# Gumo-A/hnsw_rs

Measured on AMD Instinct MI355X. Metric: queries/sec at recall@10>=0.99, 1M x 100d L2, higher is better.
Workload: dtype f32

## Files before the change

### hnsw_rs_amd/csrc/search_lean.hip

```cpp

#include <algorithm>
#include <cstdlib>

#include "device_index.h"
#include "launch.h"
#include "search_common.h"
#include "switches.h"

namespace hx {
namespace {

#define HX_LIKELY(x) __builtin_expect(!!(x), 1)
#define HX_UNLIKELY(x) __builtin_expect(!!(x), 0)

constexpr u64 LK_INVALID = ~0ull;
constexpr u64 LK_MASK = 0x7FFFFFFFFFFFFFFFull;
constexpr u64 LK_EXPANDED = 1ull << 63;

struct LeanArgs {
    const float *rows;
    const uint32_t *adj0;
    const uint32_t *adj_up;
    const uint32_t *upper_base;
    const uint32_t *ovf_off, *ovf_nbrs;
    const float *Q;
    const uint32_t *qsel;
    uint32_t *out_ids;
    float *out_dists;
    uint32_t *out_counts;
    hnsw_query_stats *out_stats;
    uint32_t n_points, ep, nb_layers, S0, S1, ef, n, slots_log2;
    unsigned long long *dbg;
    uint32_t *spill_tab;
    uint32_t spill_log2;
    uint32_t lds_limit;
};

#ifdef HX_STAMPS
__device__ __forceinline__ unsigned long long stamp_now() {
    __builtin_amdgcn_sched_barrier(0);
    asm volatile("s_waitcnt vmcnt(0) lgkmcnt(0)" ::: "memory");
    const unsigned long long t = __builtin_readcyclecounter();
    asm volatile("s_waitcnt lgkmcnt(0)" ::: "memory");
    __builtin_amdgcn_sched_barrier(0);
    return t;
}
#define STAMP(var) const unsigned long long var = stamp_now()
#define STAMP_ADD(slot, a, b) dbg_acc[slot] += (b) - (a)
#ifdef HX_STAMPS_FRONT
constexpr int HX_LEAN_DBG_SLOTS = 50;
#define FSTAMP(var) STAMP(var)
#define FSTAMP_ADD(slot, a, b) STAMP_ADD(slot, a, b)
#define FSTAMP_LDS(var)                                   \
    asm volatile("s_waitcnt lgkmcnt(0)" ::: "memory");   \
    const unsigned long long var = __builtin_readcyclecounter(); \
    asm volatile("s_waitcnt lgkmcnt(0)" ::: "memory")
#define FSTAMP_SINCE_BEGIN(slot) dbg_acc[slot] = __builtin_readcyclecounter() - t_begin
#else
constexpr int HX_LEAN_DBG_SLOTS = 40;
#endif
#define MERGE_DBG_PARAM , unsigned long long *dbg = nullptr
#define MERGE_DBG_ARG(first) , dbg_acc + (first)
#define MERGE_STAMP(var) const unsigned long long var = dbg ? stamp_now() : 0ull
#define MERGE_ADD(off, v) \
    do {                  \
        if (dbg) dbg[off] += (v); \
    } while (0)
#else
#define STAMP(var)
#define STAMP_ADD(slot, a, b)
#define MERGE_DBG_PARAM
#define MERGE_DBG_ARG(first)
#define MERGE_STAMP(var)
#define MERGE_ADD(off, v)
#endif
#if !defined(HX_STAMPS) || !defined(HX_STAMPS_FRONT)
#define FSTAMP(var)
#define FSTAMP_ADD(slot, a, b)
#define FSTAMP_LDS(var)
#define FSTAMP_SINCE_BEGIN(slot)
#endif

__device__ __forceinline__ uint32_t rdlane(uint32_t v, uint32_t l) {
    return (uint32_t)__builtin_amdgcn_readlane((int)v, (int)l);
}
__device__ __forceinline__ u64 rdlane64(u64 v, uint32_t l) {
    return ((u64)rdlane((uint32_t)(v >> 32), l) << 32) | rdlane((uint32_t)v, l);
}
__device__ __forceinline__ uint32_t uni(uint32_t x) { return (uint32_t)__builtin_amdgcn_readfirstlane((int)x); }
__device__ __forceinline__ void lds_fence() { asm volatile("s_waitcnt lgkmcnt(0)" ::: "memory"); }
template <int CTRL>
__device__ __forceinline__ uint32_t dpp_or_max(uint32_t x) {
    return (uint32_t)__builtin_amdgcn_update_dpp(-1, (int)x, CTRL, 0xF, 0xF, false);
}
__device__ __forceinline__ uint32_t wave_min_u32(uint32_t v) {
    v = min(v, dpp_or_max<0xB1>(v));
    v = min(v, dpp_or_max<0x4E>(v));
    v = min(v, dpp_or_max<0x141>(v));
    v = min(v, dpp_or_max<0x140>(v));
    return min(min(rdlane(v, 0), rdlane(v, 16)), min(rdlane(v, 32), rdlane(v, 48)));
}

struct Visited {
    uint32_t *tab;
    uint32_t bshift, bmask;

    __device__ __forceinline__ uint32_t home(uint32_t id) const { return (id * 0x9E3779B1u) >> bshift; }

    __device__ __forceinline__ uint32_t look(uint32_t id, uint32_t b) const {
        const uint4 bk = *reinterpret_cast<const uint4 *>(tab + 4 * b);
        const uint32_t m = min(min(bk.x ^ id, bk.y ^ id), min(bk.z ^ id, bk.w ^ id));
        const uint32_t nf = 4u + (uint32_t)(((int32_t)bk.x >> 31) + ((int32_t)bk.y >> 31) + ((int32_t)bk.z >> 31) +
                                            ((int32_t)bk.w >> 31));
        return m == 0 ? 4u : (nf == 4u ? 5u : nf);
    }
    __device__ __forceinline__ uint32_t claim(uint32_t id, uint32_t b, uint32_t t) const {
        uint32_t old = 0;
        if (t < 4u) old = atomicCAS(tab + 4 * b + t, HX_EMPTY_SLOT, id);
        return old;
    }
    __device__ __forceinline__ bool finish(uint32_t id, uint32_t b, uint32_t t, bool pend, bool fresh) const {
        while (__ballot(pend)) {
            if (pend) {
                if (t == 5u) b = (b + 1) & bmask;
                t = look(id, b);
                const uint32_t old = claim(id, b, t);
                const bool won = old == HX_EMPTY_SLOT;
                fresh |= won;
                pend = (t != 4u) & !won;
            }
        }
        return fresh;
    }
    __device__ __forceinline__ bool insert(uint32_t id, bool ins) const {
        const uint32_t b = home(id);
        uint32_t t = look(id, b);
        t = ins ? t : 4u;
        const uint32_t old = claim(id, b, t);
        const bool fresh = old == HX_EMPTY_SLOT;
        return finish(id, b, t, (t != 4u) & !fresh, fresh);
    }
    __device__ __forceinline__ void clear(uint32_t nslots, int lane) const {
        for (uint32_t s = lane; s < (nslots >> 2); s += 64)
            reinterpret_cast<uint4 *>(tab)[s] = make_uint4(HX_EMPTY_SLOT, HX_EMPTY_SLOT, HX_EMPTY_SLOT, HX_EMPTY_SLOT);
        lds_fence();
    }

    uint32_t *gtab = nullptr;
    uint32_t gshift = 0, gmask = 0;
    bool spill = false;

    __device__ __forceinline__ bool g_contains(uint32_t id) const {
        uint32_t s = ((id * 0x9E3779B1u) >> gshift) & gmask;
        while (true) {
            const uint32_t cur = __hip_atomic_load(gtab + s, __ATOMIC_RELAXED, __HIP_MEMORY_SCOPE_AGENT);
            if (cur == id) return true;
            if (cur == HX_EMPTY_SLOT) return false;
            s = (s + 1) & gmask;
        }
    }
    __device__ __forceinline__ uint32_t g_claim(uint32_t id) const {
        uint32_t s = ((id * 0x9E3779B1u) >> gshift) & gmask;
        while (true) {
            const uint32_t old = atomicCAS(gtab + s, HX_EMPTY_SLOT, id);
            if (old == HX_EMPTY_SLOT) return HX_EMPTY_SLOT;
            if (old == id) return id;
            s = (s + 1) & gmask;
        }
    }
    __device__ __forceinline__ void open_second_level(int lane) {
        const uint32_t nslots = gmask + 1;
        for (uint32_t s = lane; s < (nslots >> 2); s += 64)
            reinterpret_cast<uint4 *>(gtab)[s] = make_uint4(HX_EMPTY_SLOT, HX_EMPTY_SLOT, HX_EMPTY_SLOT, HX_EMPTY_SLOT);
        __builtin_amdgcn_fence(__ATOMIC_RELEASE, "agent");
        asm volatile("s_waitcnt vmcnt(0)" ::: "memory");
        spill = true;
    }
    __device__ __forceinline__ uint32_t look2(uint32_t id, uint32_t b, bool probe, bool claim_now) const {
        uint32_t t = look(id, b);
        if (!spill) return t;
        if (!probe) return 4u;
        while (t == 5u) {
            b = (b + 1) & bmask;
            t = look(id, b);
        }
        if (t == 4u) return 4u;
        if (claim_now) return g_claim(id) == HX_EMPTY_SLOT ? 7u : 4u;
        return g_contains(id) ? 4u : 6u;
    }
    __device__ __forceinline__ uint32_t claim2(uint32_t id, uint32_t b, uint32_t t) const {
        uint32_t old = 0;
        if (t < 4u)
            old = atomicCAS(tab + 4 * b + t, HX_EMPTY_SLOT, id);
        else if (t == 6u)
            old = g_claim(id);
        else if (t == 7u)
            old = HX_EMPTY_SLOT;
        return old;
    }
    __device__ __forceinline__ bool finish2(uint32_t id, uint32_t b, uint32_t t, bool pend, bool fresh) const {
        while (__ballot(pend)) {
            if (pend) {
                if (t == 5u) b = (b + 1) & bmask;
                t = look2(id, b, true, false);
                const uint32_t old = claim2(id, b, t);
                const bool won = old == HX_EMPTY_SLOT;
                fresh |= won;
                pend = (t != 4u) & !won;
            }
        }
        return fresh;
    }
};

#ifndef HX_MERGE_SHIFT_MAX
#define HX_MERGE_SHIFT_MAX 2
#endif
__device__ __forceinline__ void stage_survivors(u64 key, bool surv, u64 smask, uint32_t m, u64 *perm) {
    const uint32_t rk = __builtin_amdgcn_mbcnt_hi((uint32_t)(smask >> 32), __builtin_amdgcn_mbcnt_lo((uint32_t)smask, 0u));
    if (surv) perm[rk] = key;
    if (surv && rk + 1 == m) perm[m] = LK_INVALID;
    asm volatile("" ::: "memory");
}
template <int R>
struct Lst {
    static constexpr int NR = R;
    struct Masks {
        u64 U[R];
    };
    u64 L[R];
    uint32_t n_cur;
    u64 last_key;

    static __device__ __forceinline__ uint32_t idx_of(int r, int lane) { return (uint32_t)(R * lane + r); }
    __device__ __forceinline__ void set_first(u64 key, int lane) {
        if (lane == 0) L[0] = key;
        n_cur = 1;
    }

    __device__ __forceinline__ void init() {
#pragma unroll
        for (int r = 0; r < R; r++) L[r] = LK_INVALID;
        n_cur = 0;
        last_key = LK_INVALID;
    }
    __device__ __forceinline__ int first_unexp() const {
        uint32_t pos = 0xFFFFFFFFu;
#pragma unroll
        for (int r = 0; r < R; r++) {
            const u64 U = __ballot((int32_t)(uint32_t)(L[r] >> 32) >= 0);
            const uint32_t i = U ? (uint32_t)(R * (__ffsll((long long)U) - 1) + r) : 0xFFFFFFFFu;
            pos = min(pos, i);
        }
        return (int)pos;
    }
    __device__ __forceinline__ void unexp_masks(Masks &mk) const {
#pragma unroll
        for (int r = 0; r < R; r++) mk.U[r] = __ballot((int32_t)(uint32_t)(L[r] >> 32) >= 0);
    }
    __device__ __forceinline__ int take_first(Masks &mk) const {
        u64(&U)[R] = mk.U;
        uint32_t pos = 0xFFFFFFFFu;
#pragma unroll
        for (int r = 0; r < R; r++) {
            const uint32_t i = U[r] ? (uint32_t)(R * (__ffsll((long long)U[r]) - 1) + r) : 0xFFFFFFFFu;
            pos = min(pos, i);
        }
#pragma unroll
        for (int r = 0; r < R; r++)
            if (pos != 0xFFFFFFFFu && (pos % R) == (uint32_t)r) U[r] &= U[r] - 1;
        return (int)pos;
    }
    __device__ __forceinline__ uint32_t id_at(uint32_t pos) const {
        uint32_t v = 0;
#pragma unroll
        for (int r = 0; r < R; r++) {
            const uint32_t t = rdlane((uint32_t)L[r], pos / R);
            if ((pos % R) == (uint32_t)r) v = t;
        }
        return v;
    }
    __device__ __forceinline__ u64 key_at(uint32_t pos) const {
        u64 v = 0;
#pragma unroll
        for (int r = 0; r < R; r++) {
            const u64 t = rdlane64(L[r], pos / R);
            if ((pos % R) == (uint32_t)r) v = t;
        }
        return v;
    }
    __device__ __forceinline__ void mark(uint32_t pos, int lane) {
#pragma unroll
        for (int r = 0; r < R; r++)
            if ((pos % R) == (uint32_t)r && (uint32_t)lane == pos / R) L[r] |= LK_EXPANDED;
    }
    __device__ __forceinline__ void refresh_last(uint32_t ef) {
        last_key = n_cur >= ef ? (key_at(ef - 1) & LK_MASK) : LK_INVALID;
    }

    __device__ __forceinline__ void merge(u64 key, uint32_t ef, u64 *perm, int lane MERGE_DBG_PARAM) {
        const bool surv = key < last_key;
        const u64 smask = __ballot(surv);
        if (smask == 0) return;
        const uint32_t m = (uint32_t)__popcll(smask);
        MERGE_STAMP(m0);
        if (m <= HX_MERGE_SHIFT_MAX) {
            u64 it = smask;
            while (it) {
                const uint32_t j = (uint32_t)__ffsll((long long)it) - 1;
                it &= it - 1;
                const u64 e = rdlane64(key, j);
                const uint32_t plo = (uint32_t)__builtin_amdgcn_update_dpp(0, (int)(uint32_t)L[R - 1], 0x138, 0xF, 0xF, false);
                const uint32_t phi = (uint32_t)__builtin_amdgcn_update_dpp(0, (int)(uint32_t)(L[R - 1] >> 32), 0x138, 0xF, 0xF, false);
                const u64 below = ((u64)phi << 32) | plo;
                bool g[R];
#pragma unroll
                for (int r = 0; r < R; r++) g[r] = (L[r] & LK_MASK) > e;
                const bool gb = (below & LK_MASK) > e;
#pragma unroll
                for (int r = R - 1; r >= 0; r--) {
                    const u64 from = r > 0 ? L[r > 0 ? r - 1 : 0] : below;
                    const bool gp = r > 0 ? g[r > 0 ? r - 1 : 0] : gb;
                    L[r] = g[r] ? (gp ? from : e) : L[r];
                }
            }
            n_cur = min(n_cur + m, ef);
            if (ef < 64u * R) {
#pragma unroll
                for (int r = 0; r < R; r++)
                    if ((uint32_t)(R * lane + r) >= ef) L[r] = LK_INVALID;
            }
            refresh_last(ef);
            MERGE_STAMP(m1);
            MERGE_ADD(2, m1 - m0);
            return;
        }
        u64 *sv = perm + 64 * R;
        u64 Lm[R];
        uint32_t shift[R];
#pragma unroll
        for (int r = 0; r < R; r++) {
            Lm[r] = L[r] & LK_MASK;
            shift[r] = 0;
        }
        uint32_t srank = 0;
        stage_survivors(key, surv, smask, m, perm);
        {
            const ulonglong2 *st = reinterpret_cast<const ulonglong2 *>(perm);
            const uint32_t trips = (m + 1) >> 1;
            ulonglong2 e = st[0];
            for (uint32_t t = 1; t < trips; t++) {
                const ulonglong2 nx = st[t];
#pragma unroll
                for (int r = 0; r < R; r++) shift[r] += (e.x < Lm[r] ? 1u : 0u) + (e.y < Lm[r] ? 1u : 0u);
                srank += (e.x < key ? 1u : 0u) + (e.y < key ? 1u : 0u);
                e = nx;
            }
#pragma unroll
            for (int r = 0; r < R; r++) shift[r] += (e.x < Lm[r] ? 1u : 0u) + (e.y < Lm[r] ? 1u : 0u);
            srank += (e.x < key ? 1u : 0u) + (e.y < key ? 1u : 0u);
        }
        asm volatile("" ::: "memory");
        MERGE_STAMP(m2);
        MERGE_ADD(0, m2 - m0);
        const uint32_t n_new = min(n_cur + m, ef);
#pragma unroll
        for (int r = 0; r < R; r++) perm[R * lane + r] = LK_INVALID;
        asm volatile("" ::: "memory");
#pragma unroll
        for (int r = 0; r < R; r++) {
            const uint32_t idx = (uint32_t)(R * lane + r);
            const uint32_t np = idx + shift[r];
            if (idx < n_cur && np < n_new) perm[np] = L[r];
        }
        if (surv) sv[srank] = key;
        asm volatile("" ::: "memory");
        u64 v[R], H[R];
        bool hole[R];
#pragma unroll
        for (int r = 0; r < R; r++) v[r] = perm[R * lane + r];
#pragma unroll
        for (int r = 0; r < R; r++) {
            hole[r] = v[r] == LK_INVALID && (uint32_t)(R * lane + r) < n_new;
            H[r] = __ballot(hole[r]);
        }
#pragma unroll
        for (int r = 0; r < R; r++) {
            uint32_t hr = 0;
#pragma unroll
            for (int r2 = 0; r2 < R; r2++) {
                hr += __builtin_amdgcn_mbcnt_hi((uint32_t)(H[r2] >> 32), __builtin_amdgcn_mbcnt_lo((uint32_t)H[r2], 0u));
                if (r2 < r && hole[r2]) hr++;
            }
            if (hole[r]) v[r] = sv[hr];
        }
#pragma unroll
        for (int r = 0; r < R; r++) L[r] = v[r];
        n_cur = n_new;
        lds_fence();
        refresh_last(ef);
        MERGE_STAMP(m3);
        MERGE_ADD(1, m3 - m2);
        MERGE_ADD(3, m);
        MERGE_ADD(4, 1);
    }
};

struct LstHT {
    static constexpr int NR = 2;
    struct Masks {
        u64 head, tail;
        bool tail_known;
    };
    u64 L[2];
    uint32_t n_cur;
    u64 last_key;

    static __device__ __forceinline__ uint32_t idx_of(int r, int lane) { return (uint32_t)(64 * r + lane); }
    __device__ __forceinline__ void init() {
        L[0] = L[1] = LK_INVALID;
        n_cur = 0;
        last_key = LK_INVALID;
    }
    __device__ __forceinline__ void set_first(u64 key, int lane) {
        if (lane == 0) L[0] = key;
        n_cur = 1;
    }
    __device__ __forceinline__ void unexp_masks(Masks &mk) const {
        mk.head = __ballot((int32_t)(uint32_t)(L[0] >> 32) >= 0);
        mk.tail = 0;
        mk.tail_known = false;
    }
    __device__ __forceinline__ int take_first(Masks &mk) const {
        if (HX_LIKELY(mk.head != 0)) {
            const int pos = __ffsll((long long)mk.head) - 1;
            mk.head &= mk.head - 1;
            return pos;
        }
        if (!mk.tail_known) {
            mk.tail = n_cur > 64 ? __ballot((int32_t)(uint32_t)(L[1] >> 32) >= 0) : 0ull;
            mk.tail_known = true;
        }
        if (mk.tail == 0) return -1;
        const int pos = __ffsll((long long)mk.tail) - 1;
        mk.tail &= mk.tail - 1;
        return 64 + pos;
    }
    __device__ __forceinline__ uint32_t id_at(uint32_t pos) const {
        const uint32_t a = rdlane((uint32_t)L[0], pos & 63u), b = rdlane((uint32_t)L[1], pos & 63u);
        return pos < 64u ? a : b;
    }
    __device__ __forceinline__ u64 key_at(uint32_t pos) const {
        const u64 a = rdlane64(L[0], pos & 63u), b = rdlane64(L[1], pos & 63u);
        return pos < 64u ? a : b;
    }
    __device__ __forceinline__ void mark(uint32_t pos, int lane) {
        if ((uint32_t)lane == pos) L[0] |= LK_EXPANDED;
        if ((uint32_t)lane + 64u == pos) L[1] |= LK_EXPANDED;
    }
    __device__ __forceinline__ void refresh_last(uint32_t ef) {
        last_key = n_cur >= ef ? (rdlane64(L[1], (ef - 65u) & 63u) & LK_MASK) : LK_INVALID;
    }
    static __device__ __forceinline__ u64 shr1(u64 v) {
        const uint32_t lo = (uint32_t)__builtin_amdgcn_update_dpp(0, (int)(uint32_t)v, 0x138, 0xF, 0xF, false);
        const uint32_t hi = (uint32_t)__builtin_amdgcn_update_dpp(0, (int)(uint32_t)(v >> 32), 0x138, 0xF, 0xF, false);
        return ((u64)hi << 32) | lo;
    }
    static __device__ __forceinline__ u64 shr1_behind(u64 v, u64 w) {
        const int wlo = __builtin_amdgcn_update_dpp(0, (int)(uint32_t)w, 0x13C, 0xF, 0xF, false);
        const int whi = __builtin_amdgcn_update_dpp(0, (int)(uint32_t)(w >> 32), 0x13C, 0xF, 0xF, false);
        const uint32_t lo = (uint32_t)__builtin_amdgcn_update_dpp(wlo, (int)(uint32_t)v, 0x138, 0xF, 0xF, false);
        const uint32_t hi = (uint32_t)__builtin_amdgcn_update_dpp(whi, (int)(uint32_t)(v >> 32), 0x138, 0xF, 0xF, false);
        return ((u64)hi << 32) | lo;
    }

    __device__ __forceinline__ void merge(u64 key, uint32_t ef, u64 *perm, int lane MERGE_DBG_PARAM) {
        const bool surv = key < last_key;
        const u64 smask = __ballot(surv);
        if (smask == 0) return;
        const uint32_t m = (uint32_t)__popcll(smask);
        MERGE_STAMP(m0);
        if (m <= HX_MERGE_SHIFT_MAX) {
            u64 it = smask;
            while (it) {
                const uint32_t j = (uint32_t)__ffsll((long long)it) - 1;
                it &= it - 1;
                const u64 e = rdlane64(key, j);
                const u64 b0 = shr1(L[0]), b1 = shr1_behind(L[1], L[0]);
                const bool g0 = (L[0] & LK_MASK) > e, p0 = (b0 & LK_MASK) > e;
                const bool g1 = (L[1] & LK_MASK) > e, p1 = (b1 & LK_MASK) > e;
                L[0] = g0 ? (p0 ? b0 : e) : L[0];
                L[1] = g1 ? (p1 ? b1 : e) : L[1];
            }
            n_cur = min(n_cur + m, ef);
            if (64u + (uint32_t)lane >= ef) L[1] = LK_INVALID;
            refresh_last(ef);
            MERGE_STAMP(m1);
            MERGE_ADD(2, m1 - m0);
            return;
        }
        u64 *sv = perm + 128;
        const u64 Mm = L[0] & LK_MASK, Tm = L[1] & LK_MASK;
        uint32_t sh0 = 0, sh1 = 0, srank = 0;
        stage_survivors(key, surv, smask, m, perm);
        {
            const ulonglong2 *st = reinterpret_cast<const ulonglong2 *>(perm);
            const uint32_t trips = (m + 1) >> 1;
            ulonglong2 e = st[0];
            for (uint32_t t = 1; t < trips; t++) {
                const ulonglong2 nx = st[t];
                sh0 += (e.x < Mm ? 1u : 0u) + (e.y < Mm ? 1u : 0u);
                sh1 += (e.x < Tm ? 1u : 0u) + (e.y < Tm ? 1u : 0u);
                srank += (e.x < key ? 1u : 0u) + (e.y < key ? 1u : 0u);
                e = nx;
            }
            sh0 += (e.x < Mm ? 1u : 0u) + (e.y < Mm ? 1u : 0u);
            sh1 += (e.x < Tm ? 1u : 0u) + (e.y < Tm ? 1u : 0u);
            srank += (e.x < key ? 1u : 0u) + (e.y < key ? 1u : 0u);
        }
        asm volatile("" ::: "memory");
        MERGE_STAMP(m2);
        MERGE_ADD(0, m2 - m0);
        const uint32_t n_new = min(n_cur + m, ef);
        perm[lane] = LK_INVALID;
        perm[64 + lane] = LK_INVALID;
        asm volatile("" ::: "memory");
        {
            const uint32_t i0 = (uint32_t)lane, i1 = 64u + (uint32_t)lane;
            if (i0 < n_cur && i0 + sh0 < n_new) perm[i0 + sh0] = L[0];
            if (i1 < n_cur && i1 + sh1 < n_new) perm[i1 + sh1] = L[1];
        }
        if (surv) sv[srank] = key;
        asm volatile("" ::: "memory");
        u64 v0 = perm[lane], v1 = perm[64 + lane];
        const bool hole0 = v0 == LK_INVALID && (uint32_t)lane < n_new;
        const bool hole1 = v1 == LK_INVALID && 64u + (uint32_t)lane < n_new;
        const u64 H0 = __ballot(hole0), H1 = __ballot(hole1);
        const uint32_t hr0 = __builtin_amdgcn_mbcnt_hi((uint32_t)(H0 >> 32), __builtin_amdgcn_mbcnt_lo((uint32_t)H0, 0u));
        const uint32_t hr1 = (uint32_t)__popcll(H0) +
                             __builtin_amdgcn_mbcnt_hi((uint32_t)(H1 >> 32), __builtin_amdgcn_mbcnt_lo((uint32_t)H1, 0u));
        if (hole0) v0 = sv[hr0];
        if (hole1) v1 = sv[hr1];
        L[0] = v0;
        L[1] = v1;
        n_cur = n_new;
        lds_fence();
        refresh_last(ef);
        MERGE_STAMP(m3);
        MERGE_ADD(1, m3 - m2);
        MERGE_ADD(3, m);
        MERGE_ADD(4, 1);
    }
};

template <int DS>
__device__ __forceinline__ float chain_sum(const uint4 (&w)[DS / 4], const float (&qv)[DS]) {
    float s = 0.0f;
#pragma unroll
    for (int p = 0; p < DS / 4; p++) {
        const uint32_t dw[4] = {w[p].x, w[p].y, w[p].z, w[p].w};
#pragma unroll
        for (int j = 0; j < 4; j += 2) {
            const f32x2 x = {__builtin_bit_cast(float, dw[j]), __builtin_bit_cast(float, dw[j + 1])};
            const f32x2 y = {qv[4 * p + j], qv[4 * p + j + 1]};
            const f32x2 t = x - y;
            const f32x2 t2 = t * t;
            s += t2.x;
            s += t2.y;
        }
    }
    return s;
}
template <int DS>
__device__ __forceinline__ float row_dist(const float *rows, uint32_t id, bool want, const float (&qv)[DS]) {
    float s = 0.0f;
    if (want) {
        const uint4 *src = reinterpret_cast<const uint4 *>(rows + (size_t)id * DS);
        uint4 w[DS / 4];
#pragma unroll
        for (int p = 0; p < DS / 4; p++) w[p] = src[p];
        __builtin_amdgcn_sched_barrier(0);
        s = chain_sum<DS>(w, qv);
    }
    return __builtin_sqrtf(s);
}
__device__ __forceinline__ u64 walk_winner(uint32_t nb, bool fresh, float dist, uint32_t &j) {
    const uint32_t db = fresh ? __builtin_bit_cast(uint32_t, dist) : 0xFFFFFFFFu;
    const uint32_t mn = wave_min_u32(db);
    u64 tie = __ballot(fresh && db == mn);
    j = (uint32_t)__ffsll((long long)tie) - 1;
    uint32_t bid = rdlane(nb, j);
    tie &= tie - 1;
    while (tie) {
        const uint32_t j2 = (uint32_t)__ffsll((long long)tie) - 1;
        tie &= tie - 1;
        const uint32_t id2 = rdlane(nb, j2);
        if (id2 < bid) {
            bid = id2;
            j = j2;
        }
    }
    return ((u64)mn << 32) | bid;
}

typedef float QueryPiece __attribute__((ext_vector_type(4), aligned(4)));
template <int DS>
__device__ __forceinline__ bool load_query_f32(const float *qp, float (&qv)[DS], int lane) {
    static_assert(DS % 4 == 0 && DS / 4 <= 64, "one 16-byte piece per lane in the NaN scan");
    typedef const __attribute__((address_space(1))) QueryPiece *GlobalPieces;
    GlobalPieces src = (GlobalPieces) reinterpret_cast<const QueryPiece *>(qp);
    const QueryPiece mine = src[min(lane, DS / 4 - 1)];
    asm volatile("" : "+v"(src));
#pragma unroll
    for (int p = 0; p < DS / 4; p++) {
        const QueryPiece t = src[p];
#pragma unroll
        for (int j = 0; j < 4; j++) qv[4 * p + j] = t[j];
    }
    const bool bad = (mine[0] != mine[0]) | (mine[1] != mine[1]) | (mine[2] != mine[2]) | (mine[3] != mine[3]);
    const bool ok = __ballot(bad) == 0;
#pragma unroll
    for (int e = 0; e < DS; e++) asm volatile("" : "+v"(qv[e]));
    return ok;
}

struct TableLimits {
    uint32_t lds, all;
};
template <bool SPILLV>
__device__ __forceinline__ TableLimits layer0_table(const LeanArgs &a, Visited &vis, uint32_t hslots, uint32_t cur, int lane) {
    vis.bshift = 32 - (a.slots_log2 - 2);
    vis.bmask = (hslots >> 2) - 1;
    TableLimits lim;
    lim.lds = hslots - (hslots >> 2);
    lim.all = lim.lds;
    if constexpr (SPILLV) {
        if (a.spill_tab != nullptr) {
            if (a.lds_limit != 0) lim.lds = min(lim.lds, max(128u, a.lds_limit));
            vis.gtab = a.spill_tab + ((size_t)blockIdx.x << a.spill_log2);
            vis.gmask = (1u << a.spill_log2) - 1;
            vis.gshift = 32 - a.spill_log2;
            lim.all = lim.lds + (1u << a.spill_log2) / 2;
        }
    }
    vis.clear(hslots, lane);
    vis.insert(cur, lane == 0);
    return lim;
}

template <class LT>
__device__ __forceinline__ void write_results(const LeanArgs &a, uint32_t q, const LT &lst, uint32_t count, int lane) {
#pragma unroll
    for (int r = 0; r < LT::NR; r++) {
        const uint32_t idx = LT::idx_of(r, lane);
        if (idx < a.n) {
            const bool have = idx < count;
            a.out_ids[(size_t)q * a.n + idx] = have ? (uint32_t)lst.L[r] : HX_EMPTY_SLOT;
            if (a.out_dists)
                a.out_dists[(size_t)q * a.n + idx] =
                    have ? __builtin_bit_cast(float, (uint32_t)((lst.L[r] & LK_MASK) >> 32)) : __builtin_inff();
        }
    }
    for (uint32_t idx = 64u * LT::NR + lane; idx < a.n; idx += 64) {
        a.out_ids[(size_t)q * a.n + idx] = HX_EMPTY_SLOT;
        if (a.out_dists) a.out_dists[(size_t)q * a.n + idx] = __builtin_inff();
    }
    if (lane == 0 && a.out_counts) a.out_counts[q] = count;
}
__device__ __forceinline__ void write_stats(const LeanArgs &a, uint32_t q, uint32_t n_dist, uint32_t n_exp, uint32_t sum_deg,
                                            int32_t status, int lane) {
    if (lane == 0) {
        hnsw_query_stats st;
        st.n_dist = n_dist;
        st.n_exp = n_exp;
        st.sum_deg = sum_deg;
        st.status = status;
        a.out_stats[q] = st;
    }
}

template <int DS, class LT, int CK = 4>
__global__ void __launch_bounds__(64) hx_lean_f32_kernel(const LeanArgs a) {
    constexpr int R = LT::NR;
    static_assert(DS % 4 == 0, "whole 16-byte pieces");
    constexpr bool COOP = coop_rows<HNSW_VEC_F32, DS>();
    constexpr bool SPILLV = R >= 6;
    constexpr bool MISS_AHEAD = !COOP && !SPILLV;
    constexpr bool MISS_KEEP = MISS_AHEAD && R <= 2;
    constexpr bool WALK_AHEAD = !COOP && R <= 2;
    extern __shared__ __attribute__((aligned(16))) unsigned char smem[];
    const int lane = threadIdx.x;
    const uint32_t q = a.qsel ? a.qsel[blockIdx.x] : blockIdx.x;
    const uint32_t hslots = 1u << a.slots_log2;
    u64 *perm = reinterpret_cast<u64 *>(smem + 4ull * hslots);
    unsigned char *coop_img = reinterpret_cast<unsigned char *>(perm);
    uint32_t *coop_ids = reinterpret_cast<uint32_t *>(coop_img + HX_COOP_IMG_BYTES);
    Visited vis;
    vis.tab = reinterpret_cast<uint32_t *>(smem);

    uint32_t n_dist = 0, n_exp = 0, sum_deg = 0, n_vis = 0;
    int32_t status = HNSW_OK;
#ifdef HX_STAMPS
    unsigned long long dbg_acc[HX_LEAN_DBG_SLOTS] = {};
    const unsigned long long t_begin = __builtin_readcyclecounter();
    bool dbg_follow = false, dbg_took_pre = false;
    uint32_t dbg_pred_c = HX_EMPTY_SLOT, dbg_pred_p = HX_EMPTY_SLOT, dbg_old_p = HX_EMPTY_SLOT;
#endif

    auto row_ahead = [&](uint32_t id, uint32_t base, int layer) __attribute__((always_inline)) -> uint32_t {
        const bool up = layer >= 1, has = base != HX_EMPTY_SLOT;
        const size_t r = up ? (size_t)(has ? base : 0u) + (uint32_t)max(layer, 1) - 1 : (size_t)id;
        const uint32_t *src = (up ? a.adj_up + r * a.S1 : a.adj0 + r * a.S0) + lane;
        const bool mine = (uint32_t)lane < (up ? (has ? a.S1 : 0u) : min(a.S0, 32u));
        uint32_t v = HX_EMPTY_SLOT;
        if (mine) v = *src;
        return v;
    };
    uint32_t ub_cur = HX_EMPTY_SLOT;
    bool have_ub = false;
    if constexpr (WALK_AHEAD) {
        if (a.ep < a.n_points) {
            ub_cur = a.upper_base[a.ep];
            have_ub = true;
        }
    }

    QueryRegs<DS> qreg;
    float(&qv)[DS] = qreg.v;
    if (!load_query_f32<DS>(a.Q + (size_t)q * DS, qv, lane)) status = HNSW_ERR_NAN_INPUT;
    FSTAMP_SINCE_BEGIN(40);

    auto dist_of = [&](uint32_t id, bool want) __attribute__((always_inline)) -> float {
        if constexpr (COOP) {
            return __builtin_sqrtf(f32_rows_coop<DS, CK, true, true>(reinterpret_cast<const uint8_t *>(a.rows), id, want, qreg,
                                                                    coop_ids, coop_img, lane));
        } else {
            return row_dist<DS>(a.rows, id, want, qv);
        }
    };

    u64 best = LK_INVALID;
    uint32_t cur = a.ep;
    uint32_t row_now = HX_EMPTY_SLOT;
    if (status == HNSW_OK) {
        if (cur >= a.n_points) {
            status = HNSW_ERR_ARG;
        } else {
            if constexpr (WALK_AHEAD) row_now = row_ahead(cur, ub_cur, max((int)a.nb_layers - 1, 0));
            const float d0 = dist_of(cur, lane == 0);
            const uint32_t bits = rdlane(__builtin_bit_cast(uint32_t, d0), 0);
            n_dist = 1;
            if (__builtin_bit_cast(float, bits) != __builtin_bit_cast(float, bits))
                status = HNSW_ERR_NAN_INPUT;
            else
                best = ((u64)bits << 32) | cur;
        }
    }
    struct WalkLane {
        bool fresh;
        uint32_t ubn;
        float dist;
    };
    auto walk_eval = [&](uint32_t id, bool act) __attribute__((always_inline)) -> WalkLane {
        WalkLane r = {false, HX_EMPTY_SLOT, 0.0f};
        if constexpr (WALK_AHEAD) {
            FSTAMP(w0);
            const uint32_t vb = vis.home(id);
            const uint32_t vt0 = vis.look(id, vb);
            const uint32_t vt = act ? vt0 : 4u;
            FSTAMP(w1);
            FSTAMP_ADD(43, w0, w1);
            if (vt != 4u) {
                r.ubn = a.upper_base[id];
                const uint4 *src = reinterpret_cast<const uint4 *>(a.rows + (size_t)id * DS);
                uint4 w[DS / 4];
#pragma unroll
                for (int p = 0; p < DS / 4; p++) w[p] = src[p];
                __builtin_amdgcn_sched_barrier(0);
                const uint32_t old = vis.claim(id, vb, vt);
                r.fresh = old == HX_EMPTY_SLOT;
                const bool pend = !r.fresh;
                if (HX_UNLIKELY(__ballot(pend) != 0)) r.fresh = vis.finish(id, vb, vt, pend, r.fresh);
                __builtin_amdgcn_sched_barrier(0);
                FSTAMP_LDS(g0);
                FSTAMP(g1);
                FSTAMP_ADD(43, w1, g0);
                FSTAMP_ADD(44, g0, g1);
                r.dist = __builtin_sqrtf(chain_sum<DS>(w, qv));
                FSTAMP(g2);
                FSTAMP_ADD(45, g1, g2);
            }
        } else {
            r.fresh = vis.insert(id, act);
            if (HX_LIKELY(__ballot(r.fresh) != 0)) {
                if (r.fresh) r.ubn = a.upper_base[id];
                r.dist = dist_of(id, r.fresh);
            }
        }
        return r;
    };

#ifdef HX_STAMPS
    dbg_acc[25] = __builtin_readcyclecounter() - t_begin;
#endif
    const uint32_t up_slots = max(hslots >> 2, 64u);
    for (int layer = (int)a.nb_layers - 1; layer >= 1 && status == HNSW_OK; layer--) {
        FSTAMP(l0);
        vis.bshift = 32 - (__ffs((int)up_slots) - 1 - 2);
        vis.bmask = (up_slots >> 2) - 1;
        const uint32_t vis_limit = up_slots - (up_slots >> 2);
        vis.clear(up_slots, lane);
        vis.insert(cur, lane == 0);
        n_vis = 1;
        FSTAMP(l1);
        FSTAMP_ADD(41, l0, l1);
        if (!have_ub) {
            ub_cur = uni(a.upper_base[cur]);
            have_ub = true;
        }
        while (status == HNSW_OK) {
            if (ub_cur == HX_EMPTY_SLOT) {
                status = HNSW_ERR_NODE_NOT_IN_GRAPH;
                break;
            }
            n_exp++;
            FSTAMP_LDS(x0);
            FSTAMP(x1);
            FSTAMP_ADD(42, x0, x1);
            FSTAMP_ADD(48, 0, 1);
            bool improved = false;
            uint32_t new_cur = cur, new_ub = ub_cur;
            uint32_t ovf_lo = 0, ovf_hi = 0;
            bool first = true;
            while (true) {
                uint32_t nb = HX_EMPTY_SLOT;
                if (first) {
                    if constexpr (WALK_AHEAD) {
                        nb = row_now;
                    } else {
                        if ((uint32_t)lane < a.S1) nb = a.adj_up[((size_t)ub_cur + (uint32_t)layer - 1) * a.S1 + lane];
                    }
                } else {
                    if (ovf_lo + lane < ovf_hi) nb = a.ovf_nbrs[ovf_lo + lane];
                    ovf_lo += 64;
                }
                const bool valid = (int32_t)nb >= 0;
                if (first) {
                    const u64 pm = __ballot((int32_t)nb < 0 && nb != HX_EMPTY_SLOT);
                    if (HX_UNLIKELY(pm != 0)) {
                        const uint32_t o = rdlane(nb, (uint32_t)__ffsll((long long)pm) - 1) & ~HX_OVF_FLAG;
                        ovf_lo = uni(a.ovf_off[o]);
                        ovf_hi = uni(a.ovf_off[o + 1]);
                    }
                    first = false;
                }
                const uint32_t cnt = (uint32_t)__popcll(__ballot(valid));
                sum_deg += cnt;
                if (HX_LIKELY(cnt != 0)) {
                    if (HX_UNLIKELY(n_vis + cnt > vis_limit)) {
                        status = HNSW_ERR_OVERFLOW;
                        break;
                    }
                    const WalkLane wl = walk_eval(nb, valid);
                    const bool fresh = wl.fresh;
                    const float dist = wl.dist;
                    const u64 fm = __ballot(fresh);
                    const uint32_t nf = (uint32_t)__popcll(fm);
                    n_vis += nf;
                    n_dist += nf;
                    if (HX_LIKELY(fm != 0)) {
                        const bool nan = fresh && dist != dist;
                        if (HX_UNLIKELY(__ballot(nan) != 0)) {
                            status = HNSW_ERR_NAN_INPUT;
                            break;
                        }
                        uint32_t j;
                        const u64 k = walk_winner(nb, fresh, dist, j);
                        if (k < best) {
                            best = k;
                            new_cur = (uint32_t)k;
                            new_ub = rdlane(wl.ubn, j);
                            improved = true;
                        }
                    }
                }
                if (HX_LIKELY(ovf_lo >= ovf_hi)) break;
            }
            if (!improved || status != HNSW_OK) break;
            cur = new_cur;
            ub_cur = new_ub;
            if constexpr (WALK_AHEAD) row_now = row_ahead(cur, ub_cur, layer);
        }
        if constexpr (WALK_AHEAD) row_now = row_ahead(cur, ub_cur, layer - 1);
    }

#ifdef HX_STAMPS
    dbg_acc[7] = __builtin_readcyclecounter() - t_begin;
#endif
    const uint32_t ef = max(1u, a.ef);
    LT lst;
    lst.init();
    if (status == HNSW_OK) {
        FSTAMP(t0);
        const TableLimits lim = layer0_table<SPILLV>(a, vis, hslots, cur, lane);
        FSTAMP(t1);
        FSTAMP_ADD(47, t0, t1);
        const uint32_t lds_limit = lim.lds, vis_limit = lim.all;
        n_vis = 1;
        lst.set_first(best, lane);
        lst.refresh_last(ef);
        const uint32_t S0 = a.S0;
        const bool upper = lane >= 32;
        const uint32_t slot = (uint32_t)lane & 31u;
        uint32_t pre_nb = HX_EMPTY_SLOT, pre_c = HX_EMPTY_SLOT, pre_p = HX_EMPTY_SLOT;
        if constexpr (WALK_AHEAD) {
            pre_nb = row_now;
            pre_c = cur;
        }
        bool carry = false;
        float kdist = 0.0f;

        uint32_t ovf_lo = 0, ovf_hi = 0;

        while (true) {
            STAMP(f0);
            if constexpr (SPILLV) {
                if (HX_UNLIKELY(!vis.spill && vis.gtab != nullptr && n_vis + 64u > lds_limit)) vis.open_second_level(lane);
            }
            int ppos = -1;
            uint32_t pid = HX_EMPTY_SLOT;
            u64 pkey = 0;
            bool kept = false;
            uint32_t nb = HX_EMPTY_SLOT;
            const bool ovf_pass = ovf_lo < ovf_hi;
            if (HX_UNLIKELY(ovf_pass)) {
                if (lane < 32 && ovf_lo + (uint32_t)lane < ovf_hi) nb = a.ovf_nbrs[ovf_lo + (uint32_t)lane];
                ovf_lo += 32;
            } else {
                typename LT::Masks U;
                lst.unexp_masks(U);
                const int cpos = lst.take_first(U);
                if (HX_UNLIKELY(cpos < 0)) break;
                ppos = lst.take_first(U);
                const uint32_t cid = lst.id_at((uint32_t)cpos);
                if constexpr (MISS_AHEAD) {
                    if (ppos >= 0) {
                        pkey = lst.key_at((uint32_t)ppos);
                        pid = (uint32_t)pkey;
                    }
                } else {
                    if (ppos >= 0) pid = lst.id_at((uint32_t)ppos);
                }
                lst.mark((uint32_t)cpos, lane);
                n_exp++;
#ifdef HX_STAMPS
                if (dbg_follow) {
                    if (cid == dbg_pred_c && pid == dbg_pred_p) dbg_acc[19]++;
                    if (pid == dbg_old_p) dbg_acc[20]++;
                    dbg_follow = false;
                }
                dbg_took_pre = pre_c == cid && pre_p == pid;
#endif
                if (HX_LIKELY(pre_c == cid && pre_p == pid)) {
                    nb = pre_nb;
                    if constexpr (MISS_KEEP) kept = carry;
                } else {
                    if (slot < S0 && (!upper || ppos >= 0)) nb = a.adj0[(size_t)(upper ? pid : cid) * S0 + slot];
                }
                pre_c = HX_EMPTY_SLOT;
                carry = false;
            }
#ifdef HX_STAMPS
            asm volatile("s_waitcnt vmcnt(0)" ::: "memory");
            dbg_acc[6]++;
#endif
            STAMP(f1);
            STAMP_ADD(0, f0, f1);
#ifdef HX_STAMPS
            if (!ovf_pass && dbg_took_pre) {
                dbg_acc[21] += f1 - f0;
                dbg_acc[22]++;
            }
#endif
            const u64 pm = ovf_pass ? 0ull : __ballot((int32_t)nb < -1);
            const bool spec_ok = ppos >= 0 && (pm >> 32) == 0;
            const bool valid = (int32_t)nb >= 0 && (!upper || spec_ok);
            const uint32_t vb = vis.home(nb);
            uint32_t vt0;
            if constexpr (SPILLV)
                vt0 = vis.look2(nb, vb, valid, valid && !upper);
            else
                vt0 = vis.look(nb, vb);
            const uint32_t vt = valid ? vt0 : 4u;
            const bool want_pre = vt != 4u;
            const uint32_t ct = upper ? 4u : vt;
            bool fresh = false;
            const bool keptl = MISS_KEEP && kept && upper;
            float dist = keptl ? kdist : 0.0f;
            if constexpr (COOP) {
                const uint32_t old = SPILLV ? vis.claim2(nb, vb, ct) : vis.claim(nb, vb, ct);
                fresh = old == HX_EMPTY_SLOT;
                const bool pend = (ct != 4u) & !fresh;
                if (HX_UNLIKELY(__ballot(pend) != 0)) fresh = SPILLV ? vis.finish2(nb, vb, ct, pend, fresh) : vis.finish(nb, vb, ct, pend, fresh);
                dist = dist_of(nb, upper ? want_pre : fresh);
            } else if (want_pre && !keptl) {
                const uint4 *src = reinterpret_cast<const uint4 *>(a.rows + (size_t)nb * DS);
                uint4 w[DS / 4];
#pragma unroll
                for (int p = 0; p < DS / 4; p++) w[p] = src[p];
                __builtin_amdgcn_sched_barrier(0);
                const uint32_t old = SPILLV ? vis.claim2(nb, vb, ct) : vis.claim(nb, vb, ct);
                fresh = old == HX_EMPTY_SLOT;
                const bool pend = (ct != 4u) & !fresh;
                if (HX_UNLIKELY(__ballot(pend) != 0)) {
                    fresh = SPILLV ? vis.finish2(nb, vb, ct, pend, fresh) : vis.finish(nb, vb, ct, pend, fresh);
#ifdef HX_STAMPS
                    dbg_acc[11]++;
#endif
                }
                __builtin_amdgcn_sched_barrier(0);
#ifdef HX_STAMPS
                __builtin_amdgcn_sched_barrier(0);
                asm volatile("s_waitcnt lgkmcnt(0)" ::: "memory");
                const unsigned long long g0 = __builtin_readcyclecounter();
                asm volatile("s_waitcnt lgkmcnt(0)" ::: "memory");
                const unsigned long long g1 = stamp_now();
                dbg_acc[2] += g1 - g0;
#endif
                const float s = chain_sum<DS>(w, qv);
                dist = __builtin_sqrtf(s);
#ifdef HX_STAMPS
                asm volatile("" ::"v"(dist) : "memory");
                dbg_acc[3] += stamp_now() - g1;
#endif
            }
            const bool want = upper ? want_pre : fresh;
            const u64 vmask = __ballot(valid), fmask = __ballot(fresh);
            const uint32_t cnt_c = (uint32_t)__popcll(vmask & 0xFFFFFFFFull);
            const uint32_t cnt_p = (uint32_t)__popcll(vmask >> 32);
            const uint32_t nf_c = (uint32_t)__popcll(fmask);
            sum_deg += cnt_c;
            n_vis += nf_c;
            n_dist += nf_c;
            if (HX_UNLIKELY(n_vis > vis_limit)) {
                status = HNSW_ERR_OVERFLOW;
                break;
            }
            const bool nan = want && dist != dist;
            u64 key = LK_INVALID;
            if (want && !nan) key = ((u64)__builtin_bit_cast(uint32_t, dist) << 32) | nb;
            STAMP(f2);
            STAMP_ADD(1, f1, f2);
#ifdef HX_STAMPS
            if (kept) {
                dbg_acc[23] += f2 - f1;
                dbg_acc[24]++;
            }
#endif
            STAMP(f3);
#ifdef HX_STAMPS
            {
                const uint32_t mm = (uint32_t)__popcll(__ballot(!upper && key < lst.last_key));
                if (mm == 0) dbg_acc[12]++; else if (mm <= 2) dbg_acc[13]++; else dbg_acc[14]++;
                if (mm != 0 && mm <= HX_MERGE_SHIFT_MAX) { dbg_acc[36]++; dbg_acc[37] += mm; }
            }
#endif
            const u64 nanm = __ballot(nan);
            if (HX_UNLIKELY((nanm & 0xFFFFFFFFull) != 0)) {
                status = HNSW_ERR_NAN_INPUT;
                break;
            }
            if constexpr (MISS_AHEAD) {
                const u64 bm = __ballot(!upper && key < pkey);
                if (HX_UNLIKELY(bm != 0) && spec_ok && pm == 0) {
                    u64 k1 = rdlane64(key, (uint32_t)__ffsll((long long)bm) - 1), k2 = LK_INVALID;
                    u64 rest = bm & (bm - 1);
                    if (rest != 0) {
                        const u64 t2 = rdlane64(key, (uint32_t)__ffsll((long long)rest) - 1);
                        rest &= rest - 1;
                        k2 = max(k1, t2);
                        k1 = min(k1, t2);
                        for (int i = 2; i < 32 && rest != 0; i++) {
                            const u64 t = rdlane64(key, (uint32_t)__ffsll((long long)rest) - 1);
                            rest &= rest - 1;
                            k2 = t < k1 ? k1 : min(k2, t);
                            k1 = min(k1, t);
                        }
                    }
                    const bool again = k2 == LK_INVALID;
#ifdef HX_STAMPS
                    {
                        const uint32_t nbel = (uint32_t)__popcll(bm);
                        if (nbel == 1) dbg_acc[16]++; else if (nbel == 2) dbg_acc[17]++; else dbg_acc[18]++;
                        dbg_follow = true;
                        dbg_pred_c = (uint32_t)k1;
                        dbg_pred_p = again ? pid : (uint32_t)k2;
                        dbg_old_p = pid;
                    }
#endif
                    pre_c = (uint32_t)k1;
                    pre_p = again ? pid : (uint32_t)k2;
                    const bool held = upper && again;
                    pre_nb = held ? nb : HX_EMPTY_SLOT;
                    if (slot < S0 && !held) pre_nb = a.adj0[(size_t)(upper ? pre_p : pre_c) * S0 + slot];
                    if constexpr (MISS_KEEP) {
                        carry = again;
                        kdist = dist;
                    }
                }
            }
            lst.merge(upper ? LK_INVALID : key, ef, perm, lane MERGE_DBG_ARG(26));
            STAMP(f3b);
            STAMP_ADD(8, f3, f3b);
            if (HX_UNLIKELY((pm & 0xFFFFFFFFull) != 0)) {
                const uint32_t c_ovf = rdlane(nb, (uint32_t)__ffsll((long long)(pm & 0xFFFFFFFFull)) - 1) & ~HX_OVF_FLAG;
                ovf_lo = uni(a.ovf_off[c_ovf]);
                ovf_hi = uni(a.ovf_off[c_ovf + 1]);
                if (ovf_lo < ovf_hi) continue;
            }
            if (HX_UNLIKELY(!spec_ok)) continue;
            typename LT::Masks V;
            lst.unexp_masks(V);
            const int npos = lst.take_first(V);
            if (HX_UNLIKELY(npos < 0)) break;
            if (HX_UNLIKELY(lst.id_at((uint32_t)npos) != pid)) continue;
            {
                const int apos = lst.take_first(V);
                if (HX_LIKELY(apos >= 0)) {
                    const int bpos = lst.take_first(V);
                    pre_c = lst.id_at((uint32_t)apos);
                    pre_p = bpos >= 0 ? lst.id_at((uint32_t)bpos) : HX_EMPTY_SLOT;
                    pre_nb = HX_EMPTY_SLOT;
                    if (slot < S0 && (!upper || bpos >= 0)) pre_nb = a.adj0[(size_t)(upper ? pre_p : pre_c) * S0 + slot];
                }
            }
            STAMP(f4);
            STAMP_ADD(9, f3b, f4);
            lst.mark((uint32_t)npos, lane);
            n_exp++;
            const uint32_t pt = upper ? vt : 4u;
            const uint32_t pold = SPILLV ? vis.claim2(nb, vb, pt) : vis.claim(nb, vb, pt);
            bool pfresh = pold == HX_EMPTY_SLOT;
            const bool ppend = (pt == 5u) | ((pt < 4u) & !pfresh & (pold != nb));
            if (HX_UNLIKELY(__ballot(ppend) != 0))
                pfresh = SPILLV ? vis.finish2(nb, vb, pt == 5u ? 5u : 0u, ppend, pfresh) : vis.finish(nb, vb, pt == 5u ? 5u : 0u, ppend, pfresh);
            const uint32_t nf_p = (uint32_t)__popcll(__ballot(pfresh));
            sum_deg += cnt_p;
            n_vis += nf_p;
            n_dist += nf_p;
            if (HX_UNLIKELY(n_vis > vis_limit)) {
                status = HNSW_ERR_OVERFLOW;
                break;
            }
            if (HX_UNLIKELY(__ballot(pfresh && nan) != 0)) {
                status = HNSW_ERR_NAN_INPUT;
                break;
            }
            STAMP(f4b);
            STAMP_ADD(5, f4, f4b);
#ifdef HX_STAMPS
            {
                const uint32_t mm = (uint32_t)__popcll(__ballot(pfresh && key < lst.last_key));
                if (mm == 0) dbg_acc[12]++; else if (mm <= 2) dbg_acc[13]++; else dbg_acc[14]++;
                if (mm != 0 && mm <= HX_MERGE_SHIFT_MAX) { dbg_acc[38]++; dbg_acc[39] += mm; }
                dbg_acc[15]++;
            }
#endif
            lst.merge(pfresh ? key : LK_INVALID, ef, perm, lane MERGE_DBG_ARG(31));
            STAMP(f5);
            STAMP_ADD(10, f4b, f5);
        }
    }

    const uint32_t count = status == HNSW_OK ? min(a.n, lst.n_cur) : 0;
    write_results(a, q, lst, count, lane);
#ifdef HX_STAMPS
    if (lane == 0 && a.dbg) {
        dbg_acc[4] = __builtin_readcyclecounter() - t_begin;
        for (int i = 0; i < HX_LEAN_DBG_SLOTS; i++) a.dbg[(size_t)q * HX_LEAN_DBG_SLOTS + i] = dbg_acc[i];
    }
#endif
    write_stats(a, q, n_dist, n_exp, sum_deg, status, lane);
}

template <class LT>
__global__ void __launch_bounds__(64) hx_lean_q8_kernel(const LeanArgs a) {
    constexpr int R = LT::NR;
    constexpr bool SPILLV = R >= 6;
    constexpr int DS = 100, P = 4, NQ = 4 * (DS / 8) + DS % 8;
    constexpr uint32_t HALF = 64, ROW = 128, NCH4 = 4 * (DS / 8), REM = DS % 8;
    extern __shared__ __attribute__((aligned(16))) unsigned char smem[];
    const int lane = threadIdx.x;
    const int h = lane & 1;
    const uint32_t cslot = (uint32_t)lane >> 1;
    const uint32_t q = a.qsel ? a.qsel[blockIdx.x] : blockIdx.x;
    const uint32_t hslots = 1u << a.slots_log2;
    u64 *perm = reinterpret_cast<u64 *>(smem + 4ull * hslots);
    float *yq = reinterpret_cast<float *>(perm + 64 * R + 64);
    Visited vis;
    vis.tab = reinterpret_cast<uint32_t *>(smem);
    const uint8_t *rows8 = reinterpret_cast<const uint8_t *>(a.rows);

    uint32_t n_dist = 0, n_exp = 0, sum_deg = 0, n_vis = 0;
    int32_t status = HNSW_OK;
#ifdef HX_STAMPS
    unsigned long long dbg_acc[16] = {0, 0, 0, 0, 0, 0, 0, 0, 0, 0, 0, 0, 0, 0, 0, 0};
    const unsigned long long t_begin = __builtin_readcyclecounter();
#endif

    QRegs<NQ> qreg;
    {
        DevView dv{};
        dv.dim = DS;
        dv.half_bytes = HALF;
        dv.nch4 = NCH4;
        dv.rem = REM;
        if (!stage_query<HNSW_VEC_QUANT8>(dv, a.Q + (size_t)q * DS, yq, lane)) status = HNSW_ERR_NAN_INPUT;
#pragma unroll
        for (int e = 0; e < NQ; e++) qreg.v[e] = yq[h * (HALF - 8) + e];
    }
    auto eval = [&](uint32_t id, bool want) __attribute__((always_inline)) -> float {
        float acc[4] = {0.0f, 0.0f, 0.0f, 0.0f};
        if (want) {
            const uint4 *src = reinterpret_cast<const uint4 *>(rows8 + (size_t)id * ROW + (size_t)h * HALF);
            uint4 w[P];
#pragma unroll
            for (int p = 0; p < P; p++) w[p] = src[p];
            __builtin_amdgcn_sched_barrier(0);
            quant_half_sums<P, DS>(w, qreg, h, NCH4, REM, acc);
        }
        const float b0 = pair_swap(acc[0]), b1 = pair_swap(acc[1]), b2 = pair_swap(acc[2]), b3 = pair_swap(acc[3]);
        float s = 0.0f;
        s += acc[0];
        s += acc[1];
        s += acc[2];
        s += acc[3];
        s += b0;
        s += b1;
        s += b2;
        s += b3;
        return __builtin_sqrtf(s);
    };
    auto pair_insert = [&](uint32_t id, bool ins) __attribute__((always_inline)) -> bool {
        bool f;
        if constexpr (SPILLV) {
            const bool mine = ins && h == 0;
            const uint32_t b0 = vis.home(id);
            const uint32_t t0 = vis.look2(id, b0, mine, mine);
            const uint32_t t = mine ? t0 : 4u;
            const uint32_t old = vis.claim2(id, b0, t);
            f = old == HX_EMPTY_SLOT;
            f = vis.finish2(id, b0, t, (t != 4u) & !f, f);
        } else {
            f = vis.insert(id, ins && h == 0);
        }
        return (pair_swap_i(f ? 1 : 0) | (f ? 1 : 0)) != 0;
    };

    u64 best = LK_INVALID;
    uint32_t cur = a.ep;
    if (status == HNSW_OK) {
        if (cur >= a.n_points) {
            status = HNSW_ERR_ARG;
        } else {
            const float d0 = eval(cur, lane < 2);
            const uint32_t bits = rdlane(__builtin_bit_cast(uint32_t, d0), 0);
            n_dist = 1;
            if (__builtin_bit_cast(float, bits) != __builtin_bit_cast(float, bits))
                status = HNSW_ERR_NAN_INPUT;
            else
                best = ((u64)bits << 32) | cur;
        }
    }

    const uint32_t up_slots = max(hslots >> 2, 64u);
    uint32_t ub_cur = HX_EMPTY_SLOT;
    bool have_ub = false;
    for (int layer = (int)a.nb_layers - 1; layer >= 1 && status == HNSW_OK; layer--) {
        vis.bshift = 32 - (__ffs((int)up_slots) - 1 - 2);
        vis.bmask = (up_slots >> 2) - 1;
        const uint32_t vis_limit = up_slots - (up_slots >> 2);
        vis.clear(up_slots, lane);
        vis.insert(cur, lane == 0);
        n_vis = 1;
        if (!have_ub) {
            ub_cur = uni(a.upper_base[cur]);
            have_ub = true;
        }
        while (status == HNSW_OK) {
            if (ub_cur == HX_EMPTY_SLOT) {
                status = HNSW_ERR_NODE_NOT_IN_GRAPH;
// ... 334 lines not shown
```

Measured before the change: 6.642 million.

## Publish top-4 unexpanded frontier via LDS instead of repeated mask/take_first scans

For R<=2 non-cooperative searches, each step writes the first four unexpanded candidate keys to shared memory in one ballot/mbcnt pass and reads them back as a vector. The current, paired and prefetch candidates all come from that snapshot, replacing repeated unexp_masks/take_first/readlane scans. Nodes are marked expanded by key comparison rather than by position. The commit check now uses the foreseen-miss ballots, re-reading the frontier only when new keys land ahead of the prefetched pair. This adds LDS traffic and subtle logic-equivalence risk in exchange for fewer cross-lane scalar scans.

```diff
diff --git a/hnsw_rs_amd/csrc/search_lean.hip b/hnsw_rs_amd/csrc/search_lean.hip
--- a/hnsw_rs_amd/csrc/search_lean.hip
+++ b/hnsw_rs_amd/csrc/search_lean.hip
@@ -48,7 +48,7 @@
 #define STAMP(var) const unsigned long long var = stamp_now()
 #define STAMP_ADD(slot, a, b) dbg_acc[slot] += (b) - (a)
 #ifdef HX_STAMPS_FRONT
-constexpr int HX_LEAN_DBG_SLOTS = 50;
+constexpr int HX_LEAN_DBG_SLOTS = 53;
 #define FSTAMP(var) STAMP(var)
 #define FSTAMP_ADD(slot, a, b) STAMP_ADD(slot, a, b)
 #define FSTAMP_LDS(var)                                   \
@@ -57,7 +57,7 @@
     asm volatile("s_waitcnt lgkmcnt(0)" ::: "memory")
 #define FSTAMP_SINCE_BEGIN(slot) dbg_acc[slot] = __builtin_readcyclecounter() - t_begin
 #else
-constexpr int HX_LEAN_DBG_SLOTS = 40;
+constexpr int HX_LEAN_DBG_SLOTS = 43;
 #endif
 #define MERGE_DBG_PARAM , unsigned long long *dbg = nullptr
 #define MERGE_DBG_ARG(first) , dbg_acc + (first)
@@ -74,6 +74,9 @@
 #define MERGE_STAMP(var)
 #define MERGE_ADD(off, v)
 #endif
+#ifdef HX_STAMPS
+constexpr int HX_DBG_FRONTIER = HX_LEAN_DBG_SLOTS - 3;
+#endif
 #if !defined(HX_STAMPS) || !defined(HX_STAMPS_FRONT)
 #define FSTAMP(var)
 #define FSTAMP_ADD(slot, a, b)
@@ -222,6 +225,28 @@
     if (surv && rk + 1 == m) perm[m] = LK_INVALID;
     asm volatile("" ::: "memory");
 }
+__device__ __forceinline__ bool lk_unexp(u64 k) { return (int32_t)(uint32_t)(k >> 32) >= 0; }
+__device__ __forceinline__ uint32_t lanes_below(u64 mask, uint32_t base) {
+    return __builtin_amdgcn_mbcnt_hi((uint32_t)(mask >> 32), __builtin_amdgcn_mbcnt_lo((uint32_t)mask, base));
+}
+__device__ __forceinline__ uint32_t vpopc64(u64 mask) {
+    uint32_t r;
+    asm("v_bcnt_u32_b32 %0, %1, 0\n\tv_bcnt_u32_b32 %0, %2, %0" : "=&v"(r) : "s"((uint32_t)mask), "s"((uint32_t)(mask >> 32)));
+    return r;
+}
+__device__ __forceinline__ void frontier_publish(u64 e, bool unexp, uint32_t rank, u64 *perm, int lane) {
+    perm[(unexp && rank < 4u) ? rank : 64u + (uint32_t)lane] = e;
+}
+__device__ __forceinline__ void frontier_read(u64 (&F)[4], const u64 *perm) {
+    asm volatile("" ::: "memory");
+    const ulonglong2 *f = reinterpret_cast<const ulonglong2 *>(perm);
+    const ulonglong2 x = f[0], y = f[1];
+    F[0] = x.x;
+    F[1] = x.y;
+    F[2] = y.x;
+    F[3] = y.y;
+}
+
 template <int R>
 struct Lst {
     static constexpr int NR = R;
@@ -293,6 +318,18 @@
 #pragma unroll
         for (int r = 0; r < R; r++)
             if ((pos % R) == (uint32_t)r && (uint32_t)lane == pos / R) L[r] |= LK_EXPANDED;
+    }
+    __device__ __forceinline__ void frontier(u64 (&F)[4], u64 *perm, int lane) const {
+        static_assert(R == 1, "the interleaved lists pick by unexp_masks / take_first");
+        perm[lane] = LK_INVALID;
+        asm volatile("" ::: "memory");
+        const bool u = lk_unexp(L[0]);
+        frontier_publish(L[0], u, lanes_below(__ballot(u), 0u), perm, lane);
+        frontier_read(F, perm);
+    }
+    __device__ __forceinline__ void mark_key(u64 k) {
+#pragma unroll
+        for (int r = 0; r < R; r++) L[r] |= L[r] == k ? LK_EXPANDED : 0ull;
     }
     __device__ __forceinline__ void refresh_last(uint32_t ef) {
         last_key = n_cur >= ef ? (key_at(ef - 1) & LK_MASK) : LK_INVALID;
@@ -457,6 +494,19 @@
     __device__ __forceinline__ void mark(uint32_t pos, int lane) {
         if ((uint32_t)lane == pos) L[0] |= LK_EXPANDED;
         if ((uint32_t)lane + 64u == pos) L[1] |= LK_EXPANDED;
+    }
+    __device__ __forceinline__ void frontier(u64 (&F)[4], u64 *perm, int lane) const {
+        perm[lane] = LK_INVALID;
+        asm volatile("" ::: "memory");
+        const bool u0 = lk_unexp(L[0]), u1 = lk_unexp(L[1]);
+        const u64 B0 = __ballot(u0), B1 = __ballot(u1);
+        frontier_publish(L[0], u0, lanes_below(B0, 0u), perm, lane);
+        frontier_publish(L[1], u1, lanes_below(B1, vpopc64(B0)), perm, lane);
+        frontier_read(F, perm);
+    }
+    __device__ __forceinline__ void mark_key(u64 k) {
+        L[0] |= L[0] == k ? LK_EXPANDED : 0ull;
+        L[1] |= L[1] == k ? LK_EXPANDED : 0ull;
     }
     __device__ __forceinline__ void refresh_last(uint32_t ef) {
         last_key = n_cur >= ef ? (rdlane64(L[1], (ef - 65u) & 63u) & LK_MASK) : LK_INVALID;
@@ -688,6 +738,8 @@
     constexpr bool MISS_AHEAD = !COOP && !SPILLV;
     constexpr bool MISS_KEEP = MISS_AHEAD && R <= 2;
     constexpr bool WALK_AHEAD = !COOP && R <= 2;
+    constexpr bool FRONTIER = WALK_AHEAD;
+    static_assert(!FRONTIER || MISS_AHEAD, "the frontier's commit test is the foreseen miss's ballot");
     extern __shared__ __attribute__((aligned(16))) unsigned char smem[];
     const int lane = threadIdx.x;
     const uint32_t q = a.qsel ? a.qsel[blockIdx.x] : blockIdx.x;
@@ -927,21 +979,58 @@
             if constexpr (SPILLV) {
                 if (HX_UNLIKELY(!vis.spill && vis.gtab != nullptr && n_vis + 64u > lds_limit)) vis.open_second_level(lane);
             }
-            int ppos = -1;
+            bool has_p = false;
             uint32_t pid = HX_EMPTY_SLOT;
             u64 pkey = 0;
+            u64 akey = LK_INVALID, bkey = LK_INVALID;
             bool kept = false;
             uint32_t nb = HX_EMPTY_SLOT;
             const bool ovf_pass = ovf_lo < ovf_hi;
             if (HX_UNLIKELY(ovf_pass)) {
                 if (lane < 32 && ovf_lo + (uint32_t)lane < ovf_hi) nb = a.ovf_nbrs[ovf_lo + (uint32_t)lane];
                 ovf_lo += 32;
+            } else if constexpr (FRONTIER) {
+                u64 F[4];
+                STAMP(fr0);
+                lst.frontier(F, perm, lane);
+#ifdef HX_STAMPS
+                asm volatile("" ::"v"(F[0]), "v"(F[1]), "v"(F[2]), "v"(F[3]) : "memory");
+                dbg_acc[HX_DBG_FRONTIER] += stamp_now() - fr0;
+                dbg_acc[HX_DBG_FRONTIER + 1]++;
+#endif
+                if (HX_UNLIKELY(__ballot(lk_unexp(F[0])) == 0)) break;
+                has_p = __ballot(lk_unexp(F[1])) != 0;
+                const uint32_t cid = (uint32_t)F[0];
+                pkey = F[1];
+                pid = (uint32_t)F[1];
+                akey = F[2];
+                bkey = F[3];
+                lst.mark_key(F[0]);
+                n_exp++;
+#ifdef HX_STAMPS
+                if (dbg_follow) {
+                    if (cid == dbg_pred_c && pid == dbg_pred_p) dbg_acc[19]++;
+                    if (pid == dbg_old_p) dbg_acc[20]++;
+                    dbg_follow = false;
+                }
+                dbg_took_pre = pre_c == cid && pre_p == pid;
+#endif
+                if (HX_LIKELY(__ballot(pre_c == cid && pre_p == pid) != 0)) {
+                    nb = pre_nb;
+                    if constexpr (MISS_KEEP) kept = carry;
+                } else {
+                    if (slot < S0 && (!upper || lk_unexp(F[1]))) nb = a.adj0[(size_t)(upper ? pid : cid) * S0 + slot];
+                }
+                pre_c = HX_EMPTY_SLOT;
+                carry = false;
             } else {
+                int ppos;
                 typename LT::Masks U;
                 lst.unexp_masks(U);
                 const int cpos = lst.take_first(U);
                 if (HX_UNLIKELY(cpos < 0)) break;
                 ppos = lst.take_first(U);
+                has_p = ppos >= 0;
                 const uint32_t cid = lst.id_at((uint32_t)cpos);
                 if constexpr (MISS_AHEAD) {
                     if (ppos >= 0) {
@@ -983,7 +1072,7 @@
             }
 #endif
             const u64 pm = ovf_pass ? 0ull : __ballot((int32_t)nb < -1);
-            const bool spec_ok = ppos >= 0 && (pm >> 32) == 0;
+            const bool spec_ok = has_p && (pm >> 32) == 0;
             const bool valid = (int32_t)nb >= 0 && (!upper || spec_ok);
             const uint32_t vb = vis.home(nb);
             uint32_t vt0;
@@ -1070,8 +1159,13 @@
                 status = HNSW_ERR_NAN_INPUT;
                 break;
             }
+            u64 bm = 0;
+            u64 am = 0;
+            if constexpr (FRONTIER) {
+                am = __ballot(!upper && key < min(bkey, lst.last_key));
+            }
             if constexpr (MISS_AHEAD) {
-                const u64 bm = __ballot(!upper && key < pkey);
+                bm = __ballot(!upper && key < pkey);
                 if (HX_UNLIKELY(bm != 0) && spec_ok && pm == 0) {
                     u64 k1 = rdlane64(key, (uint32_t)__ffsll((long long)bm) - 1), k2 = LK_INVALID;
                     u64 rest = bm & (bm - 1);
@@ -1119,24 +1213,46 @@
                 if (ovf_lo < ovf_hi) continue;
             }
             if (HX_UNLIKELY(!spec_ok)) continue;
-            typename LT::Masks V;
-            lst.unexp_masks(V);
-            const int npos = lst.take_first(V);
-            if (HX_UNLIKELY(npos < 0)) break;
-            if (HX_UNLIKELY(lst.id_at((uint32_t)npos) != pid)) continue;
-            {
-                const int apos = lst.take_first(V);
-                if (HX_LIKELY(apos >= 0)) {
-                    const int bpos = lst.take_first(V);
-                    pre_c = lst.id_at((uint32_t)apos);
-                    pre_p = bpos >= 0 ? lst.id_at((uint32_t)bpos) : HX_EMPTY_SLOT;
-                    pre_nb = HX_EMPTY_SLOT;
-                    if (slot < S0 && (!upper || bpos >= 0)) pre_nb = a.adj0[(size_t)(upper ? pre_p : pre_c) * S0 + slot];
+            int npos = -1;
+            if constexpr (FRONTIER) {
+                if (HX_UNLIKELY((bm | pm) != 0)) continue;
+                if (HX_UNLIKELY(am != 0)) {
+                    u64 G[4];
+                    lst.frontier(G, perm, lane);
+                    akey = G[1];
+                    bkey = G[2];
+#ifdef HX_STAMPS
+                    dbg_acc[HX_DBG_FRONTIER + 1]++;
+                    dbg_acc[HX_DBG_FRONTIER + 2]++;
+#endif
+                }
+                pre_c = (uint32_t)akey;
+                pre_p = (uint32_t)bkey;
+                pre_nb = HX_EMPTY_SLOT;
+                if (slot < S0 && lk_unexp(upper ? bkey : akey)) pre_nb = a.adj0[(size_t)(upper ? pre_p : pre_c) * S0 + slot];
+            } else {
+                typename LT::Masks V;
+                lst.unexp_masks(V);
+                npos = lst.take_first(V);
+                if (HX_UNLIKELY(npos < 0)) break;
+                if (HX_UNLIKELY(lst.id_at((uint32_t)npos) != pid)) continue;
+                {
+                    const int apos = lst.take_first(V);
+                    if (HX_LIKELY(apos >= 0)) {
+                        const int bpos = lst.take_first(V);
+                        pre_c = lst.id_at((uint32_t)apos);
+                        pre_p = bpos >= 0 ? lst.id_at((uint32_t)bpos) : HX_EMPTY_SLOT;
+                        pre_nb = HX_EMPTY_SLOT;
+                        if (slot < S0 && (!upper || bpos >= 0)) pre_nb = a.adj0[(size_t)(upper ? pre_p : pre_c) * S0 + slot];
+                    }
                 }
             }
             STAMP(f4);
             STAMP_ADD(9, f3b, f4);
-            lst.mark((uint32_t)npos, lane);
+            if constexpr (FRONTIER)
+                lst.mark_key(pkey);
+            else
+                lst.mark((uint32_t)npos, lane);
             n_exp++;
             const uint32_t pt = upper ? vt : 4u;
             const uint32_t pold = SPILLV ? vis.claim2(nb, vb, pt) : vis.claim(nb, vb, pt);
```

Result: faster. 6.884 million, median of 6 (+3.7%).
